# sudo-monkey/fabric-token-sdk

Measured on AMD Instinct MI355X. Metric: zkatdlog transfer proofs verified/sec (node) + BN254 G1 MSM 2^20 latency, higher is better.
Workload: dtype u32 (Fp/Fr Montgomery); 1 GPU; batch verify 4096 zkatdlog transfers per GPU per step (BASELINE configs[1]); 1-GPU job of 2260992 transfers sharded by tx (configs[3]); batch_per_gpu=4096, device_pass=8192, pp=b=100,e=2, fexp=exact, parallelism=tx-sharded x1

## Files before the change

fabric-token-sdk_amd/csrc/dev/fp29.h:

```cpp
#pragma once
#include "curve.h"
#include "fp.h"
#include "fp29_const.h"

namespace fts {

struct f29 {
  int32_t l[9];
};

FTS_HD int32_t pin32(int32_t x) {
#if defined(__HIP_DEVICE_COMPILE__)
  asm volatile("" : "+v"(x));
#endif
  return x;
}
static constexpr int32_t F29_MASK = (1 << 29) - 1;

FTS_HD void pin29(f29& a) {
#pragma unroll
  for (int i = 0; i < 9; i++) a.l[i] = pin32(a.l[i]);
}

FTS_HD f29 f29_add(const f29& a, const f29& b) {
// ... 190 lines not shown
  for (int i = 0; i < 9; i++) o |= r.l[i];
  return o == 0;
}

FTS_HD f29 f29_from_fp(const fp& x) {
  f29 r;
  r.l[0] = (int32_t)((x.v[0] << 5) & (uint32_t)F29_MASK);
#pragma unroll
  for (int i = 1; i < 9; i++) {
    const int off = 29 * i - 5, w = off >> 5, s = off & 31;
    uint64_t lo = x.v[w], hi = w + 1 < 8 ? x.v[w + 1] : 0u;
    r.l[i] = (int32_t)((uint32_t)(((hi << 32) | lo) >> s) & (uint32_t)F29_MASK);
  }
  return r;
}

FTS_HD fp f29_to_fp(const f29& a) {
  f29 p29;
#pragma unroll
  for (int i = 0; i < 9; i++) p29.l[i] = P29_R256[i];
  f29 r = f29_reduce(f29_mul(a, p29));
#pragma unroll
  for (int it = 0; it < 2; it++) {
    f29 s = f29_norm(f29_add(r, fe29_p()));
    const bool take = r.l[8] < 0;
#pragma unroll
    for (int i = 0; i < 9; i++) r.l[i] = take ? s.l[i] : r.l[i];
  }
#pragma unroll
  for (int it = 0; it < 2; it++) {
    f29 s = f29_norm(f29_sub(r, fe29_p()));
    const bool take = s.l[8] >= 0;
#pragma unroll
    for (int i = 0; i < 9; i++) r.l[i] = take ? s.l[i] : r.l[i];
  }
  fp o;
#pragma unroll
  for (int j = 0; j < 8; j++) {
    const int b = 32 * j, i = b / 29, s = b % 29;
    uint64_t v = (uint64_t)(uint32_t)r.l[i] | ((uint64_t)(uint32_t)(i + 1 < 9 ? r.l[i + 1] : 0) << 29);
    if (i + 2 < 9) v |= (uint64_t)(uint32_t)r.l[i + 2] << 58;
    o.v[j] = (uint32_t)(v >> s);
  }
  return o;
}

struct q2 {
  f29 c0, c1;
};

static constexpr int32_t F29_HALF = 1 << 28;

FTS_HD int32_t f29_bdigit(int64_t acc) {
  return (int32_t)(((uint32_t)acc + (uint32_t)F29_HALF) & (uint32_t)F29_MASK) - F29_HALF;
}

FTS_HD int32_t f29_quot(int32_t t8) {
  return (int32_t)(((int64_t)t8 * P29_QMUL + ((int64_t)1 << 51)) >> 52);
}

FTS_HD f29 f29_lin2(const f29& a_, int32_t ca, const f29& b_, int32_t cb) {
  if (!__builtin_constant_p(ca)) ca = pin32(ca);
  if (!__builtin_constant_p(cb)) cb = pin32(cb);
  f29 a = a_, b = b_;
  pin29(a);
  pin29(b);
  const int32_t q = f29_quot(ca * a.l[8] + cb * b.l[8]);
  f29 r;
  int64_t acc = 0;
#pragma unroll
  for (int i = 0; i < 9; i++) {
    acc += (int64_t)ca * a.l[i] + (int64_t)cb * b.l[i] - (int64_t)q * P29B[i];
    if (i < 8) {
      const int32_t lo = f29_bdigit(acc);
      r.l[i] = lo;
      acc = (acc + F29_HALF) >> 29;
    } else {
      r.l[8] = (int32_t)acc;
    }
  }
  return r;
}

FTS_HD f29 f29_lin2_ns(const f29& a, int32_t ca, const f29& b, int32_t cb) {
  f29 r;
  int64_t acc = 0;
#pragma unroll
  for (int i = 0; i < 9; i++) {
    acc += (int64_t)ca * a.l[i] + (int64_t)cb * b.l[i];
    if (i < 8) {
      r.l[i] = f29_bdigit(acc);
      acc = (acc + F29_HALF) >> 29;
    } else {
      r.l[8] = (int32_t)acc;
    }
  }
  return r;
}

FTS_HD f29 f29_lin4(const f29& x0_, int32_t c0, const f29& x1_, int32_t c1, const f29& x2_, int32_t c2,
                    const f29& x3_, int32_t c3) {
  f29 x0 = x0_, x1 = x1_, x2 = x2_, x3 = x3_;
  pin29(x0);
  pin29(x1);
  pin29(x2);
  pin29(x3);
  c0 = pin32(c0);
  c1 = pin32(c1);
  c2 = pin32(c2);
  c3 = pin32(c3);
  const int32_t q = f29_quot(c0 * x0.l[8] + c1 * x1.l[8] + c2 * x2.l[8] + c3 * x3.l[8]);
  f29 r;
  int64_t acc = 0;
#pragma unroll
  for (int i = 0; i < 9; i++) {
    acc += (int64_t)c0 * x0.l[i] + (int64_t)c1 * x1.l[i] + (int64_t)c2 * x2.l[i] + (int64_t)c3 * x3.l[i] -
           (int64_t)q * P29B[i];
    if (i < 8) {
      r.l[i] = f29_bdigit(acc);
      acc = (acc + F29_HALF) >> 29;
    } else {
      r.l[8] = (int32_t)acc;
    }
  }
  return r;
}

FTS_HD q2 q2_neg(const q2& a) { return {f29_neg(a.c0), f29_neg(a.c1)}; }
FTS_HD q2 q2_conj(const q2& a) { return {a.c0, f29_neg(a.c1)}; }
FTS_HD q2 q2_zero() {
  q2 r;
#pragma unroll
  for (int i = 0; i < 9; i++) r.c0.l[i] = r.c1.l[i] = 0;
  return r;
}
FTS_HD q2 q2_sel(bool c, const q2& a, const q2& b) {
  q2 r;
#pragma unroll
  for (int i = 0; i < 9; i++) {
    r.c0.l[i] = c ? a.c0.l[i] : b.c0.l[i];
    r.c1.l[i] = c ? a.c1.l[i] : b.c1.l[i];
  }
  return r;
}
FTS_HD q2 q2_mul_xi(const q2& a) { return {f29_lin2(a.c0, 9, a.c1, -1), f29_lin2(a.c0, 1, a.c1, 9)}; }
FTS_HD q2 q2_mul_xi_lazy(const q2& a) { return {f29_lin2_ns(a.c0, 9, a.c1, -1), f29_lin2_ns(a.c0, 1, a.c1, 9)}; }
FTS_HD q2 q2_add(const q2& a, const q2& b) { return {f29_add(a.c0, b.c0), f29_add(a.c1, b.c1)}; }

FTS_HD f29 f29_breduce(const f29& a) { return f29_lin2(a, 1, a, 0); }

FTS_HD q2 q2_from_fp2(const fp2& a) { return {f29_breduce(f29_from_fp(a.c0)), f29_breduce(f29_from_fp(a.c1))}; }
FTS_HD fp2 q2_to_fp2(const q2& a) { return {f29_to_fp(a.c0), f29_to_fp(a.c1)}; }

struct j29 {
  f29 x, y, z;
  bool inf;
};

FTS_HD j29 j29_dbl(const j29& p) {
  f29 A = f29_sqr(p.x);
  f29 Bq = f29_sqr(p.y);
  f29 C = f29_sqr(Bq);
  f29 T2 = f29_sqr(f29_norm(f29_add(p.x, Bq)));
  f29 D1 = f29_norm(f29_sub(f29_sub(T2, A), C));
  f29 D = f29_add(D1, D1);
  f29 E = f29_norm(f29_add(f29_add(A, A), A));
  f29 F = f29_sqr(E);
  f29 X3 = f29_reduce(f29_sub(f29_norm(f29_sub(F, D)), D));
  f29 Y3a = f29_mul(E, f29_norm(f29_sub(D, X3)));
  f29 C2 = f29_add(C, C);
  f29 C4 = f29_norm(f29_add(C2, C2));
  f29 Y3 = f29_reduce(f29_sub(Y3a, f29_add(C4, C4)));
  f29 Z3 = f29_mul(f29_add(p.y, p.y), p.z);
  return {X3, Y3, Z3, p.inf};
}

FTS_HD j29 j29_madd(const j29& p, const f29& x2, const f29& y2) {
  if (p.inf) return {f29_reduce(x2), f29_reduce(y2), f29_reduce(f29_from_fp(fe_one<ModP>())), false};
  f29 Z1Z1 = f29_sqr(p.z);
  f29 U2 = f29_mul(x2, Z1Z1);
  f29 S2 = f29_mul(y2, f29_mul(p.z, Z1Z1));
  f29 H = f29_norm(f29_sub(U2, p.x));
  f29 rr = f29_sub(S2, p.y);
  f29 HH = f29_sqr(H);
  f29 HH2 = f29_add(HH, HH);
  f29 I = f29_norm(f29_add(HH2, HH2));
  f29 J = f29_mul(H, I);
  f29 r2 = f29_norm(f29_add(rr, rr));
  f29 V = f29_mul(p.x, I);
  f29 X3 = f29_reduce(f29_sub(f29_sub(f29_sub(f29_sqr(r2), J), V), V));
  f29 Y3a = f29_mul(r2, f29_norm(f29_sub(V, X3)));
  f29 YJ = f29_mul(p.y, J);
  f29 Y3 = f29_reduce(f29_sub(f29_sub(Y3a, YJ), YJ));
  f29 ZH = f29_norm(f29_add(p.z, H));
  f29 Z3 = f29_reduce(f29_sub(f29_sub(f29_sqr(ZH), Z1Z1), HH));
  if (f29_reduced_zero(Z3)) {
    if (f29_is_zero(rr)) return j29_dbl(p);
    j29 o = p;
    o.inf = true;
    return o;
  }
  return {X3, Y3, Z3, false};
}

FTS_HD j29 j29_add(const j29& p, const j29& q) {
  if (p.inf) return q;
  if (q.inf) return p;
  f29 Z1Z1 = f29_sqr(p.z);
  f29 Z2Z2 = f29_sqr(q.z);
  f29 U1 = f29_mul(p.x, Z2Z2);
  f29 U2 = f29_mul(q.x, Z1Z1);
  f29 S1 = f29_mul(p.y, f29_mul(q.z, Z2Z2));
  f29 S2 = f29_mul(q.y, f29_mul(p.z, Z1Z1));
  f29 H = f29_norm(f29_sub(U2, U1));
  f29 H2 = f29_norm(f29_add(H, H));
  f29 I = f29_sqr(H2);
  f29 J = f29_mul(H, I);
  f29 rr = f29_sub(S2, S1);
  f29 r2 = f29_norm(f29_add(rr, rr));
  f29 V = f29_mul(U1, I);
  f29 X3 = f29_reduce(f29_sub(f29_sub(f29_sub(f29_sqr(r2), J), V), V));
  f29 Y3a = f29_mul(r2, f29_norm(f29_sub(V, X3)));
  f29 SJ = f29_mul(S1, J);
  f29 Y3 = f29_reduce(f29_sub(f29_sub(Y3a, SJ), SJ));
  f29 ZZ = f29_sqr(f29_norm(f29_add(p.z, q.z)));
  f29 Z3 = f29_reduce(f29_mul(f29_norm(f29_sub(f29_sub(ZZ, Z1Z1), Z2Z2)), H));
  if (f29_reduced_zero(Z3)) {
    if (f29_is_zero(rr)) return j29_dbl(p);
    j29 o = p;
    o.inf = true;
    return o;
  }
  return {X3, Y3, Z3, false};
}

struct x29 {
  f29 x, y, zz, zzz;
  bool inf;
};

FTS_HD x29 x29_dbl_aff(const f29& x0, const f29& y0) {
  f29 x = f29_reduce(x0), y = f29_reduce(y0);
  f29 U = f29_norm(f29_add(y, y));
  f29 V = f29_sqr_c(U);
  f29 W = f29_mul_c(U, V);
  f29 S = f29_mul_c(x, V);
  f29 xx = f29_sqr_c(x);
  f29 M = f29_norm(f29_add(f29_add(xx, xx), xx));
  f29 X3 = f29_reduce(f29_sub(f29_sub(f29_sqr_c(M), S), S));
  f29 Y3 = f29_reduce(f29_sub(f29_mul_c(M, f29_norm(f29_sub(S, X3))), f29_mul_c(W, y)));
  return {X3, Y3, V, W, false};
}

FTS_HD x29 x29_madd(const x29& p, const f29& x2, const f29& y2) {
  if (p.inf) {
    f29 one = f29_reduce(f29_from_fp(fe_one<ModP>()));
    return {f29_reduce(x2), f29_reduce(y2), one, one, false};
  }
  f29 U2 = f29_mul_c(x2, p.zz);
  f29 S2 = f29_mul_c(y2, p.zzz);
  f29 P = f29_norm(f29_sub(U2, p.x));
  f29 R = f29_norm(f29_sub(S2, p.y));
  if (f29_is_zero(P)) {
    if (f29_is_zero(R)) return x29_dbl_aff(x2, y2);
    x29 o = p;
    o.inf = true;
    return o;
  }
  f29 PP = f29_sqr_c(P);
  f29 PPP = f29_mul_c(P, PP);
  f29 Q = f29_mul_c(p.x, PP);
  f29 X3 = f29_reduce(f29_sub(f29_sub(f29_sub(f29_sqr_c(R), PPP), Q), Q));
  f29 Y3a = f29_mul_c(R, f29_norm(f29_sub(Q, X3)));
  f29 Y3 = f29_reduce(f29_sub(Y3a, f29_mul_c(p.y, PPP)));
  return {X3, Y3, f29_mul_c(p.zz, PP), f29_mul_c(p.zzz, PPP), false};
}

FTS_HD j29 x29_to_j29(const x29& p) {
  if (p.inf) {
    j29 o{};
    o.inf = true;
    return o;
  }
  f29 t = f29_sqr(p.zzz);
  return {f29_mul(f29_mul(p.x, p.zz), t), f29_mul(p.y, f29_sqr(t)), f29_mul(p.zz, p.zzz), false};
}

FTS_HD j29 j29_from(const g1j& p) {
  return {f29_reduce(f29_from_fp(p.x)), f29_reduce(f29_from_fp(p.y)), f29_reduce(f29_from_fp(p.z)), is_zero(p.z)};
}
FTS_HD g1j j29_to(const j29& p) {
  if (p.inf) return jac_inf<fp>();
  return {f29_to_fp(p.x), f29_to_fp(p.y), f29_to_fp(p.z)};
}

}
```

fabric-token-sdk_amd/csrc/dev/jobs.h:

```cpp
#pragma once
#include "fp29.h"
#include "fp_wide.h"
#include "glv.h"
#include "pairing.h"
#include "sha256.h"

namespace fts {

static constexpr uint32_t NONE = 0xFFFFFFFFu;

struct G1Dev {
  uint32_t x[8], y[8];
};
struct G2Dev {
  uint32_t x0[8], x1[8], y0[8], y1[8];
};
struct F12Dev {
  uint32_t w[96];
};

enum G1Base : uint8_t { G1B_PED0 = 0, G1B_PED1, G1B_PED2, G1B_PEDGEN, G1B_GEN, G1B_COUNT };
static constexpr uint32_t G1B_SIG0 = G1B_COUNT;
static constexpr uint32_t G1B_SIG_MAX_DIGITS = (255 - G1B_SIG0) / 2;
enum G2Base : uint8_t { G2B_PK0 = 0, G2B_PK1, G2B_PK2, G2B_Q, G2B_COUNT };
// ... 335 lines not shown
  fe_to_int(out, r);
  for (int k = 0; k < 8; k++) scal[j.out][k] = out[k];
}

FTS_HD int32_t sdigit_at(const uint32_t s[8], int C, int w) {
  uint32_t carry = 0;
  int32_t d = 0;
  for (int v = 0; v <= w; v++) {
    uint32_t bit = (uint32_t)C * v, limb = bit >> 5, sh = bit & 31;
    uint64_t lo = limb < 8 ? s[limb] : 0, hi = limb + 1 < 8 ? s[limb + 1] : 0;
    uint32_t raw = (uint32_t)(((lo | (hi << 32)) >> sh) & ((1ull << C) - 1)) + carry;
    d = (int32_t)raw;
    carry = 0;
    if (raw > (1u << (C - 1))) {
      d = (int32_t)raw - (int32_t)(1u << C);
      carry = 1;
    }
  }
  return d;
}

FTS_HD g2j g2_fixed_acc(g2j acc, const G2Dev* tab, int base, const uint32_t s[8]) {
  uint32_t carry = 0;
  const G2Dev* tb = tab + (size_t)base * G2TAB_WINDOWS * G2TAB_DIGITS;
#pragma nounroll
  for (int w = 0; w < G2TAB_WINDOWS; w++) {
    uint32_t bit = (uint32_t)G2TAB_C * w, limb = bit >> 5, sh = bit & 31;
    uint64_t lo = limb < 8 ? s[limb] : 0, hi = limb + 1 < 8 ? s[limb + 1] : 0;
    uint32_t raw = (uint32_t)(((lo | (hi << 32)) >> sh) & ((1ull << G2TAB_C) - 1)) + carry;
    int32_t d = (int32_t)raw;
    carry = 0;
    if (raw > (1u << (G2TAB_C - 1))) {
      d = (int32_t)raw - (int32_t)(1u << G2TAB_C);
      carry = 1;
    }
    if (d) {
      g2a T = g2_load(tb[(size_t)w * G2TAB_DIGITS + (uint32_t)(d < 0 ? -d : d) - 1]);
      if (d < 0) T.y = f2_neg(T.y);
      acc = jac_add_aff(acc, T);
    }
  }
  return acc;
}

FTS_HD g1j g1_fixed_acc(g1j acc, const G1Dev* tab, int base, const uint32_t s[8]) {
  x29 a{};
  a.inf = is_zero(acc.z);
  if (!a.inf) {
    j29 aj = j29_from(acc);
    f29 zz = f29_sqr(aj.z);
    a = {aj.x, aj.y, zz, f29_mul(zz, aj.z), false};
  }
  uint32_t carry = 0;
  const G1Dev* tb = tab + (size_t)base * G1TAB_WINDOWS * G1TAB_DIGITS;
#pragma nounroll
  for (int w = 0; w < G1TAB_WINDOWS; w++) {
    uint32_t bit = (uint32_t)G1TAB_C * w, limb = bit >> 5, sh = bit & 31;
    uint64_t lo = limb < 8 ? s[limb] : 0, hi = limb + 1 < 8 ? s[limb + 1] : 0;
    uint32_t raw = (uint32_t)(((lo | (hi << 32)) >> sh) & ((1ull << G1TAB_C) - 1)) + carry;
    int32_t d = (int32_t)raw;
    carry = 0;
    if (raw > (1u << (G1TAB_C - 1))) {
      d = (int32_t)raw - (int32_t)(1u << G1TAB_C);
      carry = 1;
    }
    if (d) {
      g1a T = g1_load(tb[(size_t)w * G1TAB_DIGITS + (uint32_t)(d < 0 ? -d : d) - 1]);
      f29 y = f29_from_fp(T.y);
      a = x29_madd(a, f29_from_fp(T.x), d < 0 ? f29_neg(y) : y);
    }
  }
  return j29_to(x29_to_j29(a));
}

FTS_HD g1j g1_mul_glv(const g1a& p, const uint32_t k[8]) {
  g1j acc = jac_inf<fp>();
  if (p.inf) return acc;
  uint32_t k1[4], k2[4];
  bool n1, n2;
  glv_split(k, k1, n1, k2, n2);
  g1a P1 = n1 ? aff_neg(p) : p;
  g1a P2;
  P2.x = p.x * fe_const<ModP>(GLV_BETA);
  P2.y = n2 ? fe_neg(p.y) : p.y;
  P2.inf = false;
  g1j Sj = jac_add_aff(jac_from_aff(P1), P2);
  fp z2 = sqr(Sj.z), z3 = z2 * Sj.z;
  P1.x = P1.x * z2;
  P1.y = P1.y * z3;
  P2.x = P2.x * z2;
  P2.y = P2.y * z3;
  g1a S;
  S.x = Sj.x;
  S.y = Sj.y;
  S.inf = false;
  uint32_t u0 = k1[0], u1 = k1[1], u2 = k1[2], u3 = k1[3];
  uint32_t v0 = k2[0], v1 = k2[1], v2 = k2[2], v3 = k2[3];
#pragma nounroll
  for (int i = 127; i >= 0; i--) {
    acc = jac_dbl(acc);
    uint32_t b1 = u3 >> 31, b2 = v3 >> 31;
    u3 = (u3 << 1) | (u2 >> 31);
    u2 = (u2 << 1) | (u1 >> 31);
    u1 = (u1 << 1) | (u0 >> 31);
    u0 <<= 1;
    v3 = (v3 << 1) | (v2 >> 31);
    v2 = (v2 << 1) | (v1 >> 31);
    v1 = (v1 << 1) | (v0 >> 31);
    v0 <<= 1;
    g1a T;
    T.x = b1 ? (b2 ? S.x : P1.x) : P2.x;
    T.y = b1 ? (b2 ? S.y : P1.y) : P2.y;
    T.inf = false;
    g1j nacc = jac_add_aff(acc, T);
    if (b1 | b2) acc = nacc;
  }
  acc.z = acc.z * Sj.z;
  return acc;
}

FTS_HD int booth16(const uint32_t k[4], int i) {
  int pos = 4 * i - 1;
  uint32_t v;
  if (pos < 0) {
    v = (k[0] << 1) & 31u;
  } else {
    int l = pos >> 5, o = pos & 31;
    uint32_t lo = l == 0 ? k[0] : (l == 1 ? k[1] : (l == 2 ? k[2] : (l == 3 ? k[3] : 0u)));
    uint32_t hi = l == 0 ? k[1] : (l == 1 ? k[2] : (l == 2 ? k[3] : 0u));
    v = (uint32_t)(((((uint64_t)hi) << 32) | lo) >> o) & 31u;
  }
  return (int)(v & 1u) + (int)((v >> 1) & 7u) - 8 * (int)(v >> 4);
}

FTS_HD void g1dev_put(G1Dev& d, const fp& a, const fp& b) {
#pragma unroll
  for (int q = 0; q < 8; q++) {
    d.x[q] = a.v[q];
    d.y[q] = b.v[q];
  }
}
FTS_HD void g1dev_get(const G1Dev& d, fp& a, fp& b) {
#pragma unroll
  for (int q = 0; q < 8; q++) {
    a.v[q] = d.x[q];
    b.v[q] = d.y[q];
  }
}
FTS_HD g1j g1_mul_glv16_iso(const g1a& p, const fp& zin, const uint32_t k[8], G1Dev* tb, size_t st);
FTS_HD g1j g1_mul_glv16(const g1a& p, const uint32_t k[8], G1Dev* tb, size_t st) {
  if (p.inf) return jac_inf<fp>();
  return g1_mul_glv16_iso(p, fe_one<ModP>(), k, tb, st);
}
FTS_HD g1j g1_mul_glv16_iso(const g1a& p, const fp& zin, const uint32_t k[8], G1Dev* tb, size_t st) {
  g1j acc = jac_inf<fp>();
  uint32_t k1[4], k2[4];
  bool n1, n2;
  glv_split(k, k1, n1, k2, n2);
  g1a P1 = n1 ? aff_neg(p) : p;
  g1j T = jac_from_aff(P1);
  fp pre = fe_one<ModP>();
#pragma nounroll
  for (int e = 0; e < 8; e++) {
    if (e == 1) T = jac_dbl(T);
    if (e >= 2) T = jac_add_aff(T, P1);
    g1dev_put(tb[e * st], T.x, T.y);
    g1dev_put(tb[(8 + e) * st], T.z, pre);
    pre = pre * T.z;
  }
  const fp Zc = pre;
  fp suf = fe_one<ModP>();
#pragma nounroll
  for (int e = 7; e >= 0; e--) {
    fp X, Y, Z, pe;
    g1dev_get(tb[e * st], X, Y);
    g1dev_get(tb[(8 + e) * st], Z, pe);
    fp se = pe * suf;
    fp s2 = sqr(se);
    suf = suf * Z;
    g1dev_put(tb[e * st], X * s2, Y * (s2 * se));
  }
  const bool flip = n1 != n2;
  const f29 beta29 = f29_reduce(f29_from_fp(fe_const<ModP>(GLV_BETA)));
  j29 a = {f29{}, f29{}, f29{}, true};
#pragma nounroll
  for (int i = 32; i >= 0; i--) {
    int d1 = booth16(k1, i), d2 = booth16(k2, i);
    int m1 = d1 < 0 ? -d1 : d1, m2 = d2 < 0 ? -d2 : d2;
    fp x1, y1, x2, y2;
    g1dev_get(tb[(size_t)(m1 ? m1 - 1 : 0) * st], x1, y1);
    g1dev_get(tb[(size_t)(m2 ? m2 - 1 : 0) * st], x2, y2);
    if (i != 32) {
      a = j29_dbl(a);
      a = j29_dbl(a);
      a = j29_dbl(a);
      a = j29_dbl(a);
    }
    f29 Y = f29_from_fp(y1);
    j29 na = j29_madd(a, f29_from_fp(x1), (d1 < 0) ? f29_neg(Y) : Y);
    if (m1) a = na;
    Y = f29_from_fp(y2);
    na = j29_madd(a, f29_mul(f29_from_fp(x2), beta29), ((d2 < 0) != flip) ? f29_neg(Y) : Y);
    if (m2) a = na;
  }
  acc = j29_to(a);
  acc.z = acc.z * (Zc * zin);
  return acc;
}

FTS_HD void g1_emit_bytes(const G1Job& j, const g1a& r, uint8_t* arena) {
  if (j.bytes != NONE) g1_to_bytes_g(arena + j.bytes, r);
  if (j.b64 != NONE) {
    uint8_t tmp[64];
    g1_to_bytes(tmp, r);
    b64_encode_64(arena + j.b64, tmp);
  }
}

struct G1JDev {
  uint32_t x[8], y[8], z[8];
};
FTS_HD void g1j_store(G1JDev& d, const g1j& p) {
#pragma unroll
  for (int i = 0; i < 8; i++) {
    d.x[i] = p.x.v[i];
    d.y[i] = p.y.v[i];
    d.z[i] = p.z.v[i];
  }
}
FTS_HD g1j g1j_load(const G1JDev& d) {
  g1j p;
#pragma unroll
  for (int i = 0; i < 8; i++) {
    p.x.v[i] = d.x[i];
    p.y.v[i] = d.y[i];
    p.z.v[i] = d.z[i];
  }
  return p;
}

FTS_HD uint64_t vterm_w(const VTerm& v) { return ((uint64_t)v.w_hi << 32) | v.w_lo; }
FTS_HD g1j g1_var_point(const G1Job& j, const VTerm* vterms, const G1Dev* pts) {
  const VTerm& v0 = vterms[j.vstart];
  const uint64_t b = vterm_w(v0);
  const bool horner = (v0.flags & VT_HORNER) != 0;
  if (j.vcount == 1 && (horner || b == 1) && !(v0.flags & VT_NEG)) return jac_from_aff(g1_load(pts[v0.pt]));
  if (horner && (b & (b - 1)) == 0) {
    const int top = b ? 63 - __builtin_clzll(b) : 0;
    g1j V = jac_from_aff(g1_load(pts[v0.pt]));
    for (uint32_t t = 1; t < j.vcount; t++) {
#pragma nounroll
      for (int q = 0; q < top; q++) V = jac_dbl(V);
      V = jac_add_aff(V, g1_load(pts[vterms[j.vstart + t].pt]));
    }
    return b ? V : jac_from_aff(g1_load(pts[vterms[j.vstart + j.vcount - 1].pt]));
  }
  uint64_t cmax = 0;
  if (horner) {
    cmax = 1;
    for (uint32_t t = 1; t < j.vcount; t++) cmax *= b;
  } else {
    for (uint32_t t = 0; t < j.vcount; t++) cmax |= vterm_w(vterms[j.vstart + t]);
  }
  g1j V = jac_inf<fp>();
  if (cmax == 0) return V;
  const int top = 63 - __builtin_clzll(cmax);
#pragma nounroll
  for (int q = top; q >= 0; q--) {
    if (q != top) V = jac_dbl(V);
    uint64_t c = 1;
#pragma nounroll
    for (uint32_t t = j.vcount; t-- > 0;) {
      const VTerm& vt = vterms[j.vstart + t];
      const uint64_t w = horner ? c : vterm_w(vt);
      if ((w >> q) & 1) {
        const g1a P = g1_load(pts[vt.pt]);
        V = jac_add_aff(V, (vt.flags & VT_NEG) ? aff_neg(P) : P);
      }
      c *= b;
    }
  }
  return V;
}

FTS_HD void job_g1(const G1Job& j, const VTerm* vterms, const G1Dev* pts, const uint32_t (*scal)[8],
                   const G1Dev* tab, G1Dev* g1out, uint8_t* arena) {
  g1j acc = jac_inf<fp>();
  if (j.vscal != NONE) {
    g1j V = g1_var_point(j, vterms, pts);
    if (j.vneg) V = jac_neg(V);
    G1Dev loc[16];
    if (!is_zero(V.z)) acc = g1_mul_glv16_iso(g1a{V.x, V.y, false}, V.z, scal[j.vscal], loc, 1);
  }
  for (int f = 0; f < j.nfix; f++) acc = g1_fixed_acc(acc, tab, j.fbase[f], scal[j.fscal[f]]);
  g1a r = jac_to_aff(acc);
  G1Dev d;
  g1_store(d, r);
  g1out[j.out] = d;
  g1_emit_bytes(j, r, arena);
}

FTS_HD void job_g1_part(const G1Job* jobs, uint32_t n, uint32_t i, const VTerm* vterms, const G1Dev* pts,
                        const uint32_t (*scal)[8], const G1Dev* tab, G1JDev* part, G1Dev* vtab) {
  uint32_t f = i / n, jb = i - f * n;
  const G1Job& j = jobs[jb];
  if (f == 3 && j.sh_count) return;
  g1j acc = jac_inf<fp>();
  if (f < 3) {
    if (f < j.nfix) acc = g1_fixed_acc(acc, tab, j.fbase[f], scal[j.fscal[f]]);
  } else if (j.vscal != NONE) {
    g1j V = g1_var_point(j, vterms, pts);
    if (j.vneg) V = jac_neg(V);
#if defined(__HIP_DEVICE_COMPILE__)
    G1Dev* tb = vtab + jb;
    const size_t st = n;
#else
    G1Dev loc[16];
    G1Dev* tb = vtab ? vtab + jb : loc;
    const size_t st = vtab ? n : 1;
#endif
    if (!is_zero(V.z)) acc = g1_mul_glv16_iso(g1a{V.x, V.y, false}, V.z, scal[j.vscal], tb, st);
  }
  g1j_store(part[i], acc);
}

FTS_HD g1j job_g1_sum_parts(const G1Job& j, uint32_t jb, uint32_t n, const G1JDev* part) {
  g1j acc = jac_inf<fp>();
  if (j.sh_count) {
    acc = g1j_load(part[3 * (size_t)n + j.sh_first]);
    for (uint32_t s = 1; s < j.sh_count; s++) acc = jac_add(acc, g1j_load(part[3 * (size_t)n + j.sh_first + s]));
  } else if (j.vscal != NONE) {
    acc = g1j_load(part[3 * (size_t)n + jb]);
  }
  for (uint32_t f = 0; f < 3; f++)
    if (f < j.nfix) acc = jac_add(acc, g1j_load(part[(size_t)f * n + jb]));
  return acc;
}

FTS_HD void job_g1_finish(const G1Job& j, const g1j& acc, const fp& zi, G1Dev* g1out, uint8_t* arena) {
  g1a r;
  r.inf = is_zero(acc.z);
  fp zi2 = sqr(zi);
  r.x = r.inf ? fe_zero<ModP>() : acc.x * zi2;
  r.y = r.inf ? fe_zero<ModP>() : acc.y * zi2 * zi;
  G1Dev d;
  g1_store(d, r);
  g1out[j.out] = d;
  g1_emit_bytes(j, r, arena);
}

FTS_HD void g1_pnorm(const g1j& acc, const fp& inv, G1Dev& out) {
  fp z2 = sqr(acc.z);
  G1Dev d;
  g1_store(d, g1a{acc.x * z2 * inv, sqr(z2) * inv, false});
  out = d;
// ... 355 lines not shown
```

fabric-token-sdk_amd/csrc/dev/msm.h:

```cpp
#pragma once
#include "jobs.h"

namespace fts {

struct MsmPlan {
  uint32_t n;
  uint32_t glv;
  uint32_t nv;
  uint32_t c;
  uint32_t windows;
  uint32_t buckets;
  uint32_t slot_cap;
  uint32_t seg_len;
  uint32_t max_slots;
  uint32_t segs;
  uint32_t pre;
  uint32_t rw;
  uint32_t per;
  uint32_t pts;
  uint64_t nv_magic;
};

static constexpr uint32_t MSM_TREE_CHUNK = 128;
static constexpr uint32_t MSM_SEG_THREADS = 128;
// ... 60 lines not shown
    uint64_t tot = (uint64_t)p.rw * p.max_slots;
    seg_len = 4;
    while (seg_len < 64 && tot / (2 * seg_len) >= 65536) seg_len *= 2;
  }
  p.seg_len = seg_len;
  p.segs = (p.max_slots + seg_len - 1) / seg_len;
  return p;
}

FTS_HD int32_t msm_digit(const uint32_t k[8], uint32_t c, uint32_t w, uint32_t& carry) {
  uint32_t bit = c * w, limb = bit >> 5, sh = bit & 31;
  uint64_t lo = limb < 8 ? k[limb] : 0, hi = limb + 1 < 8 ? k[limb + 1] : 0;
  uint32_t raw = (uint32_t)(((lo | (hi << 32)) >> sh) & ((1ull << c) - 1)) + carry;
  if (raw > (1u << (c - 1))) {
    carry = 1;
    return (int32_t)raw - (int32_t)(1u << c);
  }
  carry = 0;
  return (int32_t)raw;
}

static constexpr uint32_t MSM_ZERO = 0x40000000u;
static constexpr uint32_t MSM_T_MASK = 0x3FFFFFFFu;

FTS_HD uint32_t msm_key_bits(const MsmPlan& p) { return p.c > 1 ? p.c - 1 : 1; }

FTS_HD void msm_put_key(const MsmPlan& p, uint32_t w, uint32_t vi, int32_t d, bool neg, uint32_t* key,
                        uint32_t* val) {
  size_t t = (size_t)w * p.nv + vi;
  if (d == 0) {
    key[t] = 0;
    val[t] = p.pre ? p.pts - 1 : (uint32_t)t | MSM_ZERO;
    return;
  }
  key[t] = (uint32_t)(d < 0 ? -d : d) - 1;
  val[t] = (uint32_t)t | (((d < 0) != neg) ? 0x80000000u : 0u);
}

FTS_HD void msm_job_keys(const MsmPlan& p, uint32_t i, const uint32_t (*scal)[8], uint32_t* key, uint32_t* val) {
  if (p.glv) {
    uint32_t k1[4], k2[4];
    bool n1, n2;
    glv_split(scal[i], k1, n1, k2, n2);
    uint32_t a[8] = {k1[0], k1[1], k1[2], k1[3], 0, 0, 0, 0}, b[8] = {k2[0], k2[1], k2[2], k2[3], 0, 0, 0, 0};
    uint32_t ca = 0, cb = 0;
    for (uint32_t w = 0; w < p.windows; w++) {
      msm_put_key(p, w, i, msm_digit(a, p.c, w, ca), n1, key, val);
      msm_put_key(p, w, p.n + i, msm_digit(b, p.c, w, cb), n2, key, val);
    }
  } else {
    uint32_t carry = 0;
    for (uint32_t w = 0; w < p.windows; w++) msm_put_key(p, w, i, msm_digit(scal[i], p.c, w, carry), false, key, val);
  }
}

FTS_HD uint32_t msm_window_of(const MsmPlan& p, uint32_t x) {
  uint32_t w = (uint32_t)(((uint64_t)x * p.nv_magic) >> 32);
  return (uint64_t)w * p.nv > x ? w - 1 : w;
}

FTS_HD uint32_t msm_entry_bucket(const MsmPlan& p, uint64_t t, const uint32_t* skey, const uint32_t* sval) {
  if (p.pre) return skey[t];
  return msm_window_of(p, sval[t] & MSM_T_MASK) * p.buckets + skey[t];
}

FTS_HD void msm_job_bounds(const MsmPlan& p, uint64_t t, uint64_t total, const uint32_t* skey, const uint32_t* sval,
                           uint32_t* start, uint32_t* end) {
  uint32_t g = msm_entry_bucket(p, t, skey, sval);
  if (t == 0) start[g] = 0;
  if (t + 1 == total) {
    end[g] = (uint32_t)total;
    return;
  }
  uint32_t g1 = msm_entry_bucket(p, t + 1, skey, sval);
  if (g1 != g) {
    end[g] = (uint32_t)(t + 1);
    start[g1] = (uint32_t)(t + 1);
  }
}

FTS_HD void msm_job_phi(const MsmPlan& p, uint32_t i, G1Dev* pts) {
  g1a P = g1_load(pts[i]);
  if (!P.inf) P.x = P.x * fe_const<ModP>(GLV_BETA);
  G1Dev d;
  g1_store(d, P);
  pts[p.n + i] = d;
}

FTS_HD void msm_job_precompute(const MsmPlan& p, uint32_t v, G1Dev* pts) {
  g1a P = g1_load(pts[v]);
  g1j acc = {P.x, P.y, fe_one<ModP>()};
  for (uint32_t w = 1; w < p.windows; w++) {
    g1a r;
    r.inf = P.inf;
    if (!P.inf) {
      for (uint32_t q = 0; q < p.c; q++) acc = jac_dbl(acc);
      fp zi = fp_inv_var(acc.z), zi2 = sqr(zi);
      r.x = acc.x * zi2;
      r.y = acc.y * zi2 * zi;
    }
    G1Dev d;
    g1_store(d, r);
    pts[(size_t)w * p.nv + v] = d;
  }
}

FTS_HD uint32_t msm_bucket_slots(const MsmPlan& p, uint32_t count) {
  uint32_t m = (count + p.slot_cap - 1) / p.slot_cap;
  return m ? m : 1;
}

FTS_HD void msm_job_owner(const MsmPlan& p, uint32_t g, const uint32_t* count, const uint32_t* soff,
                          uint32_t* owner, uint32_t* wlo, uint32_t* whi) {
  uint32_t m = msm_bucket_slots(p, count[g]), o = soff[g];
  for (uint32_t s = 0; s < m; s++) owner[o + s] = g;
  uint32_t w = g / p.buckets, b = g - w * p.buckets;
  if (b == 0) wlo[w] = o;
  if (b == p.buckets - 1) whi[w] = o + m;
}

FTS_HD uint32_t msm_slot_len(const MsmPlan& p, uint32_t j, const uint32_t* owner, const uint32_t* soff,
                             const uint32_t* count) {
  uint32_t g = owner[j], s = j - soff[g], lo = s * p.slot_cap, hi = lo + p.slot_cap;
  if (hi > count[g]) hi = count[g];
  return hi > lo ? hi - lo : 0;
}

FTS_HD g1j msm_job_slot(const MsmPlan& p, uint32_t j, const uint32_t* owner, const uint32_t* soff,
                        const uint32_t* start, const uint32_t* count, const uint32_t* perm, const G1Dev* pts) {
  uint32_t g = owner[j], s = j - soff[g];
  uint32_t lo = s * p.slot_cap, hi = lo + p.slot_cap;
  if (hi > count[g]) hi = count[g];
  const uint32_t* e = perm + start[g];
  g1j acc = jac_inf<fp>();
  if (lo >= hi) return acc;
  const uint32_t base = p.pre ? 0u : (g / p.buckets) * p.nv, ident = p.pts - 1;
  auto point_of = [&](uint32_t v) -> uint32_t {
    return p.pre ? (v & 0x7FFFFFFFu) : ((v & MSM_ZERO) ? ident : (v & MSM_T_MASK) - base);
  };
  uint32_t v = e[lo];
  G1Dev nxt = pts[point_of(v)];
  x29 a{};
  a.inf = true;
  for (uint32_t q = lo; q < hi; q++) {
    G1Dev cur = nxt;
    uint32_t sign = v >> 31;
    if (q + 1 < hi) {
      v = e[q + 1];
      nxt = pts[point_of(v)];
    }
    g1a P = g1_load(cur);
    if (!P.inf) {
      f29 Y = f29_from_fp(P.y);
      a = x29_madd(a, f29_from_fp(P.x), sign ? f29_neg(Y) : Y);
    }
  }
  return j29_to(x29_to_j29(a));
}

FTS_HD j29 j29_inf() {
  j29 o{};
  o.inf = true;
  return o;
}
FTS_HD j29 j29_ld(const G1JDev& d) { return j29_from(g1j_load(d)); }

FTS_HD j29 j29_mul_small(const j29& p, uint32_t k) {
  if (!k) return j29_inf();
  const j29 p2 = j29_dbl(p), p3 = j29_add(p2, p);
  const int top = 31 - __builtin_clz(k), w = top >> 1;
  uint32_t d = (k >> (2 * w)) & 3u;
  j29 acc = d == 1 ? p : (d == 2 ? p2 : p3);
  for (int i = w - 1; i >= 0; i--) {
    acc = j29_dbl(j29_dbl(acc));
    d = (k >> (2 * i)) & 3u;
    if (d) acc = j29_add(acc, d == 1 ? p : (d == 2 ? p2 : p3));
  }
  return acc;
}

FTS_HD g1j msm_job_segment(const MsmPlan& p, uint32_t w, uint32_t s, const uint32_t* wlo, const uint32_t* whi,
                           const uint32_t* owner, const G1JDev* slot_sum) {
  uint32_t lo = wlo[w] + s * p.seg_len, hi = lo + p.seg_len;
  if (hi > whi[w]) hi = whi[w];
  if (lo >= hi) return jac_inf<fp>();
  j29 run = j29_inf(), acc = j29_inf();
  for (uint32_t j = hi; j > lo; j--) {
    run = j29_add(run, j29_ld(slot_sum[j - 1]));
    if (j - 1 == lo || owner[j - 2] != owner[j - 1]) acc = j29_add(acc, run);
  }
  uint32_t bl = owner[lo] - w * p.buckets;
  return j29_to(j29_add(acc, j29_mul_small(run, bl)));
}

FTS_HD bool g1_from_raw(const uint8_t* b, g1a& a) {
  uint32_t x[8], y[8], t[8], mm[8];
  be32_to_limbs(x, b);
  be32_to_limbs(y, b + 32);
  for (int q = 0; q < 8; q++) mm[q] = P_MOD[q];
  bool canon = ((b[0] & 0xC0) == 0) && sub8(t, x, mm) && sub8(t, y, mm);
  a.x = fe_from_int<ModP>(x);
  a.y = fe_from_int<ModP>(y);
  a.inf = is_zero(a.x) && is_zero(a.y);
  return canon && g1_on_curve(a);
}

FTS_HD void g1j_to_raw(const g1j& acc, uint8_t out[64]) {
  g1a r;
  r.inf = is_zero(acc.z);
  fp zi = r.inf ? fe_one<ModP>() : fp_inv_var(acc.z), zi2 = sqr(zi);
  r.x = r.inf ? fe_zero<ModP>() : acc.x * zi2;
  r.y = r.inf ? fe_zero<ModP>() : acc.y * zi2 * zi;
  g1_to_bytes(out, r);
}

FTS_HDN uint32_t g1_sum_raw(uint32_t n, const uint8_t* raw, uint8_t out[64]) {
  g1j acc = jac_inf<fp>();
  for (uint32_t i = 0; i < n; i++) {
    g1a a;
    if (!g1_from_raw(raw + 64 * (size_t)i, a)) return i;
    acc = jac_add_aff(acc, a);
  }
  g1j_to_raw(acc, out);
  return n;
}

}
```

Measured before the change: 949,300 transfers/s.

## Use fused lazy-reduction Montgomery scans in G1 Jacobian double and mixed add

Adds a column-wise Montgomery product scan over the 29-bit limb representation that fuses multiply, square, sum-of-products and add-after-reduce into a single reduction pass. j29_dbl and j29_madd are rewritten to use fewer normalisations and reductions, and doubling uses a halving-by-3/2 trick with a cheaper formula. x29_madd gets a fused variant while the MSM bucket path keeps the old version under a new name. This cuts reductions and limb normalisations in the GLV scalar multiplication used by proof verification. The risk is limb-bound overflow or correctness problems from the looser reduction.

```diff
diff --git a/fabric-token-sdk_amd/csrc/dev/fp29.h b/fabric-token-sdk_amd/csrc/dev/fp29.h
--- a/fabric-token-sdk_amd/csrc/dev/fp29.h
+++ b/fabric-token-sdk_amd/csrc/dev/fp29.h
@@ -366,50 +366,111 @@
 FTS_HD q2 q2_from_fp2(const fp2& a) { return {f29_breduce(f29_from_fp(a.c0)), f29_breduce(f29_from_fp(a.c1))}; }
 FTS_HD fp2 q2_to_fp2(const q2& a) { return {f29_to_fp(a.c0), f29_to_fp(a.c1)}; }
 
+enum { S29_NONE = 0, S29_MUL = 1, S29_SQR = 2 };
+
+template <int KIND>
+FTS_HD void s29_col(int64_t& acc, const f29& a, const f29& b, const f29& b2, int k) {
+  if (KIND == S29_MUL) {
+#pragma unroll
+    for (int i = 0; i < 9; i++) {
+      const int j = k - i;
+      if (j < 0 || j > 8) continue;
+      acc += (int64_t)a.l[i] * b.l[j];
+    }
+  } else if (KIND == S29_SQR) {
+#pragma unroll
+    for (int i = 0; i < 9; i++) {
+      const int j = k - i;
+      if (j <= i || j > 8) continue;
+      acc += (int64_t)b2.l[i] * a.l[j];
+    }
+    if ((k & 1) == 0) acc += (int64_t)b.l[k / 2] * a.l[k / 2];
+  }
+}
+
+template <int K1, int K2, bool ADD>
+FTS_HD f29 s29_scan(const f29& a, const f29& b, const f29& c, const f29& d, const f29& f) {
+  FTS_COUNT_MAD(64 * ((K1 != S29_NONE) + (K2 != S29_NONE)) + 72);
+  const f29 b2 = K1 == S29_SQR ? f29_add(b, b) : b, d2 = K2 == S29_SQR ? f29_add(d, d) : d;
+  int64_t acc = 0;
+  int32_t m[9];
+  f29 r;
+#pragma unroll
+  for (int k = 0; k < 17; k++) {
+    s29_col<K1>(acc, a, b, b2, k);
+    s29_col<K2>(acc, c, d, d2, k);
+#pragma unroll
+    for (int i = 0; i < 9; i++) {
+      const int j = k - i;
+      if (i >= k || j < 0 || j > 8) continue;
+      acc += (int64_t)m[i] * P29B[j];
+    }
+    if (k < 9) {
+      const uint32_t m0 = ((uint32_t)acc * P29_INV) & (uint32_t)F29_MASK;
+      m[k] = (int32_t)((m0 + (uint32_t)F29_HALF) & (uint32_t)F29_MASK) - F29_HALF;
+      acc = (acc + (int64_t)m[k] * P29B[0]) >> 29;
+    } else {
+      if (ADD) acc += f.l[k - 9];
+      r.l[k - 9] = f29_bdigit(acc);
+      acc = (acc + F29_HALF) >> 29;
+    }
+  }
+  r.l[8] = (int32_t)acc + (ADD ? f.l[8] : 0);
+  return r;
+}
+
+FTS_HD f29 s29_mul(const f29& a, const f29& b) { return s29_scan<S29_MUL, S29_NONE, false>(a, b, a, a, a); }
+FTS_HD f29 s29_sqr(const f29& a) { return s29_scan<S29_SQR, S29_NONE, false>(a, a, a, a, a); }
+FTS_HD f29 s29_sqr_add(const f29& a, const f29& f) { return s29_scan<S29_SQR, S29_NONE, true>(a, a, a, a, f); }
+FTS_HD f29 s29_mul2(const f29& a, const f29& b, const f29& c, const f29& d) {
+  return s29_scan<S29_MUL, S29_MUL, false>(a, b, c, d, a);
+}
+FTS_HD f29 s29_mul_sub_sqr(const f29& a, const f29& b, const f29& c) {
+  return s29_scan<S29_MUL, S29_SQR, false>(a, b, c, f29_neg(c), a);
+}
+
+FTS_HD f29 f29_half3(const f29& a) {
+  const int32_t odd = -(a.l[0] & 1);
+  int32_t v[9];
+#pragma unroll
+  for (int i = 0; i < 9; i++) v[i] = 3 * a.l[i] + (odd & P29B[i]);
+  f29 r;
+#pragma unroll
+  for (int i = 0; i < 8; i++) r.l[i] = (v[i] >> 1) + ((v[i + 1] & 1) << 28);
+  r.l[8] = v[8] >> 1;
+  return r;
+}
+
 struct j29 {
   f29 x, y, z;
   bool inf;
 };
 
 FTS_HD j29 j29_dbl(const j29& p) {
-  f29 A = f29_sqr(p.x);
-  f29 Bq = f29_sqr(p.y);
-  f29 C = f29_sqr(Bq);
-  f29 T2 = f29_sqr(f29_norm(f29_add(p.x, Bq)));
-  f29 D1 = f29_norm(f29_sub(f29_sub(T2, A), C));
-  f29 D = f29_add(D1, D1);
-  f29 E = f29_norm(f29_add(f29_add(A, A), A));
-  f29 F = f29_sqr(E);
-  f29 X3 = f29_reduce(f29_sub(f29_norm(f29_sub(F, D)), D));
-  f29 Y3a = f29_mul(E, f29_norm(f29_sub(D, X3)));
-  f29 C2 = f29_add(C, C);
-  f29 C4 = f29_norm(f29_add(C2, C2));
-  f29 Y3 = f29_reduce(f29_sub(Y3a, f29_add(C4, C4)));
-  f29 Z3 = f29_mul(f29_add(p.y, p.y), p.z);
+  const f29 T = s29_sqr(p.y);
+  const f29 Z3 = s29_mul(p.y, p.z);
+  const f29 S = s29_mul(p.x, T);
+  const f29 M = f29_half3(s29_sqr(p.x));
+  const f29 X3 = s29_sqr_add(M, f29_neg(f29_add(S, S)));
+  const f29 Y3 = s29_mul_sub_sqr(M, f29_sub(S, X3), T);
   return {X3, Y3, Z3, p.inf};
 }
 
 FTS_HD j29 j29_madd(const j29& p, const f29& x2, const f29& y2) {
-  if (p.inf) return {f29_reduce(x2), f29_reduce(y2), f29_reduce(f29_from_fp(fe_one<ModP>())), false};
-  f29 Z1Z1 = f29_sqr(p.z);
-  f29 U2 = f29_mul(x2, Z1Z1);
-  f29 S2 = f29_mul(y2, f29_mul(p.z, Z1Z1));
-  f29 H = f29_norm(f29_sub(U2, p.x));
-  f29 rr = f29_sub(S2, p.y);
-  f29 HH = f29_sqr(H);
-  f29 HH2 = f29_add(HH, HH);
-  f29 I = f29_norm(f29_add(HH2, HH2));
-  f29 J = f29_mul(H, I);
-  f29 r2 = f29_norm(f29_add(rr, rr));
-  f29 V = f29_mul(p.x, I);
-  f29 X3 = f29_reduce(f29_sub(f29_sub(f29_sub(f29_sqr(r2), J), V), V));
-  f29 Y3a = f29_mul(r2, f29_norm(f29_sub(V, X3)));
-  f29 YJ = f29_mul(p.y, J);
-  f29 Y3 = f29_reduce(f29_sub(f29_sub(Y3a, YJ), YJ));
-  f29 ZH = f29_norm(f29_add(p.z, H));
-  f29 Z3 = f29_reduce(f29_sub(f29_sub(f29_sqr(ZH), Z1Z1), HH));
+  if (p.inf) return {f29_breduce(x2), f29_breduce(y2), f29_breduce(f29_from_fp(fe_one<ModP>())), false};
+  const f29 Z1Z1 = s29_sqr(p.z);
+  const f29 U2 = s29_mul(x2, Z1Z1);
+  const f29 S2 = s29_mul(y2, s29_mul(p.z, Z1Z1));
+  const f29 H = f29_sub(U2, p.x);
+  const f29 Z3 = s29_mul(p.z, H);
+  const f29 rr = f29_sub(S2, p.y);
+  const f29 HH = s29_sqr(H);
+  const f29 HHH = s29_mul(H, HH);
+  const f29 V = s29_mul(p.x, HH);
+  const f29 X3 = s29_sqr_add(rr, f29_neg(f29_add(HHH, f29_add(V, V))));
+  const f29 Y3 = s29_mul2(rr, f29_sub(V, X3), f29_neg(p.y), HHH);
   if (f29_reduced_zero(Z3)) {
-    if (f29_is_zero(rr)) return j29_dbl(p);
+    if (f29_reduced_zero(f29_breduce(rr))) return j29_dbl(p);
     j29 o = p;
     o.inf = true;
     return o;
@@ -468,6 +529,38 @@
 
 FTS_HD x29 x29_madd(const x29& p, const f29& x2, const f29& y2) {
   if (p.inf) {
+    const f29 one = f29_breduce(f29_from_fp(fe_one<ModP>()));
+    return {f29_breduce(x2), f29_breduce(y2), one, one, false};
+  }
+  const f29 U2 = s29_mul(x2, p.zz);
+  const f29 S2 = s29_mul(y2, p.zzz);
+  const f29 P = f29_sub(U2, p.x);
+  const f29 R = f29_sub(S2, p.y);
+  const f29 PP = s29_sqr(P);
+  const f29 ZZ3 = s29_mul(p.zz, PP);
+  f29 Pq = P, PPq = PP, Rq = R, X1 = p.x, nY1 = f29_neg(p.y), ZZZ1 = p.zzz;
+  pin29(Pq);
+  pin29(PPq);
+  pin29(Rq);
+  pin29(X1);
+  pin29(nY1);
+  pin29(ZZZ1);
+  const f29 PPP = s29_mul(Pq, PPq);
+  const f29 ZZZ3 = s29_mul(ZZZ1, PPP);
+  const f29 Q = s29_mul(X1, PPq);
+  const f29 X3 = s29_sqr_add(Rq, f29_neg(f29_add(PPP, f29_add(Q, Q))));
+  const f29 Y3 = s29_mul2(Rq, f29_sub(Q, X3), nY1, PPP);
+  if (f29_reduced_zero(ZZ3)) {
+    if (f29_reduced_zero(f29_breduce(Rq))) return x29_dbl_aff(x2, y2);
+    x29 o = p;
+    o.inf = true;
+    return o;
+  }
+  return {X3, Y3, ZZ3, ZZZ3, false};
+}
+
+FTS_HD x29 x29_madd_c(const x29& p, const f29& x2, const f29& y2) {
+  if (p.inf) {
     f29 one = f29_reduce(f29_from_fp(fe_one<ModP>()));
     return {f29_reduce(x2), f29_reduce(y2), one, one, false};
   }
diff --git a/fabric-token-sdk_amd/csrc/dev/jobs.h b/fabric-token-sdk_amd/csrc/dev/jobs.h
--- a/fabric-token-sdk_amd/csrc/dev/jobs.h
+++ b/fabric-token-sdk_amd/csrc/dev/jobs.h
@@ -511,11 +511,17 @@
   if (p.inf) return jac_inf<fp>();
   return g1_mul_glv16_iso(p, fe_one<ModP>(), k, tb, st);
 }
+FTS_HD g1j g1_mul_glv16_halves(const g1a& p, const fp& zin, const uint32_t k1[4], bool n1, const uint32_t k2[4],
+                               bool n2, G1Dev* tb, size_t st);
 FTS_HD g1j g1_mul_glv16_iso(const g1a& p, const fp& zin, const uint32_t k[8], G1Dev* tb, size_t st) {
-  g1j acc = jac_inf<fp>();
   uint32_t k1[4], k2[4];
   bool n1, n2;
   glv_split(k, k1, n1, k2, n2);
+  return g1_mul_glv16_halves(p, zin, k1, n1, k2, n2, tb, st);
+}
+FTS_HD g1j g1_mul_glv16_halves(const g1a& p, const fp& zin, const uint32_t k1[4], bool n1, const uint32_t k2[4],
+                               bool n2, G1Dev* tb, size_t st) {
+  g1j acc = jac_inf<fp>();
   g1a P1 = n1 ? aff_neg(p) : p;
   g1j T = jac_from_aff(P1);
   fp pre = fe_one<ModP>();
@@ -559,7 +565,7 @@
     j29 na = j29_madd(a, f29_from_fp(x1), (d1 < 0) ? f29_neg(Y) : Y);
     if (m1) a = na;
     Y = f29_from_fp(y2);
-    na = j29_madd(a, f29_mul(f29_from_fp(x2), beta29), ((d2 < 0) != flip) ? f29_neg(Y) : Y);
+    na = j29_madd(a, s29_mul(f29_from_fp(x2), beta29), ((d2 < 0) != flip) ? f29_neg(Y) : Y);
     if (m2) a = na;
   }
   acc = j29_to(a);
diff --git a/fabric-token-sdk_amd/csrc/dev/msm.h b/fabric-token-sdk_amd/csrc/dev/msm.h
--- a/fabric-token-sdk_amd/csrc/dev/msm.h
+++ b/fabric-token-sdk_amd/csrc/dev/msm.h
@@ -236,7 +236,7 @@
     g1a P = g1_load(cur);
     if (!P.inf) {
       f29 Y = f29_from_fp(P.y);
-      a = x29_madd(a, f29_from_fp(P.x), sign ? f29_neg(Y) : Y);
+      a = x29_madd_c(a, f29_from_fp(P.x), sign ? f29_neg(Y) : Y);
     }
   }
   return j29_to(x29_to_j29(a));
```

After: 979,300 transfers/s (median of 6 runs). +3.2%, better.
